# GloryyrolG/MHEntropy

Hardware: AMD Instinct MI355X
Metric: hypotheses/sec (BxK) fwd+loss, 256x256 (higher is better)
Workload: dtype bf16; 1 GPU; c2: MHEnt.get_loss forward+loss, resnet50 encoder (train-mode BN), 12-coupling RealNVP h=512, MANO joints, B=256/GPU, K=64, 256x256; images_per_gpu=256, hypotheses_per_image=64, global_batch=256, launch=hip-graph replay, base_noise=drawn on the device inside the step (Philox4x32-10, mhe_randn_f32), timing=one window of 452 steps, bracketed by barrier + synchronize, ranks=1, rccl_ranks=0

## Files before the change

### mhentropy_amd/csrc/conv_halo.hip

```cpp
#include "conv_shared.h"

#ifndef MHE_HALO_ABL
#define MHE_HALO_ABL 0
#endif

namespace mhe { namespace conv {

namespace {

typedef unsigned u4 __attribute__((ext_vector_type(4)));
typedef __attribute__((ext_vector_type(8))) __bf16 bf8;
typedef float v16f __attribute__((ext_vector_type(16)));

constexpr int HBM = 256, HBN = 128;
constexpr int H_STAGE = 16384, H_RING = 4;
constexpr int H_MAXC = 512;
constexpr unsigned H_OOB = 0x80000000u;

template <int W> struct Geo {
    static constexpr int R = HBM / W;
    static constexpr int PW = W + 2, HP = (R + 2) * PW;
    static constexpr int HALO = HP * 128;
    static constexpr int NP = HP * 8;
    static constexpr int NJ = (NP + 255) / 256;
};

}

template <int W, bool DG>
__global__ __launch_bounds__(768) void conv_halo_kernel(const Params p) {
    using T = u16;
    using G = Geo<W>;
    constexpr int R = G::R, PW = G::PW, HALO = G::HALO, NP = G::NP, NJ = G::NJ;
    static_assert(NJ <= 12, "six load steps of two pieces");
    __shared__ uint4 lds[(H_RING * H_STAGE + 2 * HALO) / 16];
    __shared__ float aff[3 * H_MAXC];
    unsigned char *const ring = reinterpret_cast<unsigned char *>(lds), *const halo0 = ring + H_RING * H_STAGE;
    const int tid = threadIdx.x, lane = tid & 63, wave = __builtin_amdgcn_readfirstlane(tid >> 6);
    const int C = p.Cin, nC = C / 64, Tn = nC * 9;
    const int gm = p.M / HBM, gn = p.Cout / HBN, ntiles = gm * gn;
    const int TPI = p.H / R;
    auto tile_at = [&](int L, int &mt, int &nt) __attribute__((always_inline)) {
        if (gn > 1 && (gm & 7) == 0) {
            const int slot = L >> 3;
            nt = slot % gn;
            mt = (slot / gn) * 8 + (L & 7);
        } else { mt = L % gm; nt = L / gm; }
    };
    const bool bn = p.in_scale != nullptr;
    const bool rev = DG && p.rev_coef != nullptr;
    if (rev) for (int i = tid; i < C; i += 768) { aff[i] = p.rev_coef[i]; aff[H_MAXC + i] = p.rev_coef[C + i]; aff[2 * H_MAXC + i] = p.rev_coef[2 * C + i]; }
    constexpr int abl = MHE_HALO_ABL;
    if (bn) for (int i = tid; i < C; i += 768) { aff[i] = p.in_scale[i]; aff[H_MAXC + i] = p.in_shift[i]; }
    const int nbar_epi = (MHE_HALO_ABL & 16) ? 3 : 3 + (!DG && p.stats ? 2 : 0) + (DG && BN_EPILOGUE && p.bn_y[0] ? 2 : 0);
    __syncthreads();

    if (wave < 8) {
        const int l31 = lane & 31, kg = lane >> 5;
        const int wm = wave >> 1, wn = wave & 1;
        int hpb[2], xcb[2];
#pragma unroll
        for (int mt = 0; mt < 2; ++mt) {
            const int pm = wm * 64 + mt * 32 + l31;
            hpb[mt] = (pm / W + 1) * PW + (pm % W) + 1;
            xcb[mt] = (pm % W) + 1;
        }
        const size_t wbytes = (size_t)gn * Tn * H_STAGE;
        const u4 rsw = {(unsigned)(size_t)p.w, (unsigned)((size_t)p.w >> 32) & 0xffffu, (unsigned)wbytes, 0x00020000u};
        const unsigned ring_lds = (unsigned)(size_t)((__attribute__((address_space(3))) unsigned char *)ring);
        int gc = 0;
        for (int L = blockIdx.x; L < ntiles; L += (int)gridDim.x) {
            int mtile, ntile;
            tile_at(L, mtile, ntile);
            auto issue = [&](int tau) __attribute__((always_inline)) {
                const unsigned off = tau < Tn ? (unsigned)((ntile * Tn + tau) * H_STAGE + wave * 2048 + lane * 16) : H_OOB;
                const unsigned off1 = tau < Tn ? off + 1024u : H_OOB;
                const unsigned lb = ring_lds + (unsigned)((tau & 3) * H_STAGE + wave * 2048);
                unsigned keep;
                asm volatile("s_mov_b32 %[keep], m0\n\ts_mov_b32 m0, %[lb]\n\ts_nop 0\n\tbuffer_load_dwordx4 %[v0], %[rs], 0 offen lds\n\t"
                             "s_add_u32 m0, %[lb], 1024\n\ts_nop 0\n\tbuffer_load_dwordx4 %[v1], %[rs], 0 offen lds\n\ts_mov_b32 m0, %[keep]"
                             : [keep] "=&s"(keep) : [v0] "v"(off), [v1] "v"(off1), [rs] "s"(rsw), [lb] "s"(lb) : "memory");
            };
            v16f acc[2][2];
#pragma unroll
            for (int a = 0; a < 2; ++a)
#pragma unroll
                for (int b = 0; b < 2; ++b)
#pragma unroll
                    for (int i = 0; i < 16; ++i) acc[a][b][i] = 0.f;
            if constexpr (!(abl & 4)) { issue(0); issue(1); issue(2); }
            __builtin_amdgcn_s_barrier();
            __builtin_amdgcn_sched_barrier(0);
            for (int c = 0; c < nC; ++c) {
                const unsigned char *hb = halo0 + ((gc + c) & 1) * HALO;
#pragma unroll
                for (int tap = 0; tap < 9; ++tap) {
                    const int tau = c * 9 + tap;
                    asm volatile("s_waitcnt vmcnt(4)" ::: "memory");
                    __builtin_amdgcn_s_barrier();
                    __builtin_amdgcn_sched_barrier(0);
                    if constexpr (!(abl & 4)) issue(tau + 3);
                    if constexpr (abl & 2) continue;
                    const unsigned char *ws = ring + ((c + tap) & 3) * H_STAGE + (wn * 8) * 1024 + lane * 16;
                    const int toff = (tap / 3 - 1) * PW + (tap % 3 - 1);
                    const unsigned char *ha[2];
                    int fx[2];
#pragma unroll
                    for (int mt = 0; mt < 2; ++mt) {
                        int hp0 = hpb[mt];
                        asm volatile("" : "+v"(hp0));
                        const int hp = hp0 + toff;
                        ha[mt] = hb + hp * 128;
                        fx[mt] = (kg ^ (((xcb[mt] + (tap % 3 - 1)) >> 1) & 7)) << 4;
                    }
#pragma unroll
                    for (int ks = 0; ks < 4; ++ks) {
                        uint4 fb[2], fa[2];
#pragma unroll
                        for (int nt = 0; nt < 2; ++nt) fb[nt] = *reinterpret_cast<const uint4 *>(ws + (nt * 4 + ks) * 1024);
#pragma unroll
                        for (int mt = 0; mt < 2; ++mt) fa[mt] = *reinterpret_cast<const uint4 *>(ha[mt] + (fx[mt] ^ (ks << 5)));
#pragma unroll
                        for (int nt = 0; nt < 2; ++nt)
#pragma unroll
                            for (int mt = 0; mt < 2; ++mt)
                                if constexpr (abl & 1) acc[nt][mt][0] += __uint_as_float((fb[nt].x ^ fa[mt].x) + (fb[nt].w ^ fa[mt].w));
                                else acc[nt][mt] = __builtin_amdgcn_mfma_f32_32x32x16_bf16(__builtin_bit_cast(bf8, fb[nt]), __builtin_bit_cast(bf8, fa[mt]),
                                                                                           acc[nt][mt], 0, 0, 0);
                    }
                }
            }
            gc += nC;
            asm volatile("s_waitcnt vmcnt(0)" ::: "memory");
            __builtin_amdgcn_s_barrier();
            __builtin_amdgcn_sched_barrier(0);
#pragma unroll
            for (int nt = 0; nt < 2; ++nt)
#pragma unroll
                for (int mt = 0; mt < 2; ++mt)
#pragma unroll
                    for (int b = 0; b < 4; ++b) {
                        const int row = wm * 64 + mt * 32 + l31, boff = (wn * 64 + nt * 32 + 8 * b + 4 * kg) * 2;
                        const int chunk = (boff >> 4) ^ (row & 15);
                        uint2 o;
                        o.x = (unsigned)f32_to_bf16(acc[nt][mt][4 * b]) | ((unsigned)f32_to_bf16(acc[nt][mt][4 * b + 1]) << 16);
                        o.y = (unsigned)f32_to_bf16(acc[nt][mt][4 * b + 2]) | ((unsigned)f32_to_bf16(acc[nt][mt][4 * b + 3]) << 16);
                        *reinterpret_cast<uint2 *>(ring + ((size_t)row * 16 + chunk) * 16 + (boff & 15)) = o;
                    }
            __syncthreads();
            const int m0 = mtile * HBM;
            if constexpr (!(abl & 16)) epilogue_store<T, HBM, HBN, 512, DG, 2, 1>(p, ring, mtile % NSH, ntile * HBN, [&](int row) { return (long)(m0 + row); });
            __syncthreads();
        }
    } else {
        const int tr = tid - 512;
        const T *xg = reinterpret_cast<const T *>(p.x);
        auto locate = [&](int j, int rb, int r1, int cc, long &goff, int &lo, bool &inner) __attribute__((always_inline)) {
            int trv = tr;
            asm volatile("" : "+v"(trv));
            const int e = trv + 256 * j;
            if (e >= NP) { goff = -2; lo = 0; inner = false; return; }
            const int hp = e >> 3, slot = e & 7, hr = hp / PW, hc = hp - hr * PW;
            const int col = hc - 1;
            lo = hp * 128 + ((slot ^ ((hc >> 1) & 7)) << 4);
            const bool ok = (unsigned)(r1 + hr) < (unsigned)p.H && (unsigned)col < (unsigned)W;
            goff = ok ? ((long)(rb + hr) * W + col) * C + cc * 64 + slot * 8 : -1l;
            inner = ok && hr >= 1 && hr <= R;
        };
        uint4 regs[NJ], regs2[DG ? NJ : 1];
        const T *x2g = reinterpret_cast<const T *>(p.x2);
        const int slot8 = (tr & 7) * 8;
        float sc[8], sh[8], k0[DG ? 8 : 1];
        auto affine_of = [&](int cc) __attribute__((always_inline)) {
#pragma unroll
            for (int i = 0; i < 8; ++i) { sc[i] = aff[cc * 64 + slot8 + i]; sh[i] = aff[H_MAXC + cc * 64 + slot8 + i]; }
            if constexpr (DG) {
#pragma unroll
                for (int i = 0; i < 8; ++i) k0[i] = aff[2 * H_MAXC + cc * 64 + slot8 + i];
            }
        };
        auto load_all = [&](int rb, int r1, int cc) __attribute__((always_inline)) {
#pragma unroll
            for (int j = 0; j < NJ; ++j) {
                long goff; int lo; bool inner;
                locate(j, rb, r1, cc, goff, lo, inner);
                regs[j] = goff >= 0 ? *reinterpret_cast<const uint4 *>(xg + goff) : make_uint4(0u, 0u, 0u, 0u);
                if constexpr (DG) { if (rev) regs2[j] = goff >= 0 ? *reinterpret_cast<const uint4 *>(x2g + goff) : make_uint4(0u, 0u, 0u, 0u); }
            }
        };
        auto store2 = [&](int s, int rb, int r1, int cc, unsigned char *hb, T *ag) __attribute__((always_inline)) {
#pragma unroll
            for (int i = 0; i < 2; ++i) {
                const int j = 2 * s + i;
                if (j >= NJ) continue;
                long goff; int lo; bool inner;
                locate(j, rb, r1, cc, goff, lo, inner);
                if (goff == -2) continue;
                uint4 v = regs[j];
                if (bn && goff >= 0) {
                    float f[8];
                    Chunk<T>::unpack(v, f);
#pragma unroll
                    for (int k = 0; k < 8; ++k) { f[k] = fmaf(f[k], sc[k], sh[k]); if (p.relu_in) f[k] = fmaxf(f[k], 0.f); }
                    v = Chunk<T>::pack(f);
                }
                if constexpr (DG) {
                    if (rev && goff >= 0) {
                        float f[8], y[8];
                        Chunk<T>::unpack(v, f);
                        Chunk<T>::unpack(regs2[j], y);
#pragma unroll
                        for (int k = 0; k < 8; ++k) f[k] = fmaf(sc[k], f[k], fmaf(sh[k], y[k], k0[k]));
                        v = Chunk<T>::pack(f);
                    }
                }
                *reinterpret_cast<uint4 *>(hb + lo) = v;
                if (ag && inner) *reinterpret_cast<uint4 *>(ag + goff) = v;
            }
        };
        int gc = 0;
        {
            int mt0, nt0;
            tile_at(blockIdx.x, mt0, nt0);
            T *ag = p.a_out && nt0 == 0 ? reinterpret_cast<T *>(p.a_out) : nullptr;
            const int r1 = (mt0 % TPI) * R - 1, rb = (mt0 / TPI) * p.H + r1;
            if (bn || rev) affine_of(0);
            load_all(rb, r1, 0);
#pragma unroll
            for (int s = 0; s < 6; ++s) store2(s, rb, r1, 0, halo0, ag);
        }
        for (int L = blockIdx.x; L < ntiles; L += (int)gridDim.x) {
            int mtile, ntile;
            tile_at(L, mtile, ntile);
            for (int c = 0; c < nC; ++c) {
                int mt2 = mtile, nt2 = ntile, c2 = c + 1;
                bool have = true;
                if (c2 == nC) {
                    c2 = 0;
                    have = L + (int)gridDim.x < ntiles;
                    if (have) tile_at(L + (int)gridDim.x, mt2, nt2);
                }
                unsigned char *hb = halo0 + ((gc + c + 1) & 1) * HALO;
                T *ag = p.a_out && nt2 == 0 ? reinterpret_cast<T *>(p.a_out) : nullptr;
                const int r1 = (mt2 % TPI) * R - 1, rb = (mt2 / TPI) * p.H + r1;
                if (c == 0) {
                    asm volatile("s_waitcnt lgkmcnt(0)" ::: "memory");
                    __builtin_amdgcn_s_barrier();
                    __builtin_amdgcn_sched_barrier(0);
                }
#pragma unroll
                for (int s = 0; s < 9; ++s) {
                    if (have && !(abl & 8)) {
                        if (s == 0) { load_all(rb, r1, c2); if (bn || rev) affine_of(c2); }
                        if (s >= 3) store2(s - 3, rb, r1, c2, hb, ag);
                    }
                    asm volatile("s_waitcnt lgkmcnt(0)" ::: "memory");
                    __builtin_amdgcn_s_barrier();
                    __builtin_amdgcn_sched_barrier(0);
                }
            }
            gc += nC;
            asm volatile("s_waitcnt lgkmcnt(0)" ::: "memory");
            for (int i = 0; i < nbar_epi; ++i) __builtin_amdgcn_s_barrier();
        }
    }
}

bool halo_supports(const Params &p) {
    return p.KH == 3 && p.KW == 3 && p.stride == 1 && p.pad == 1 && (p.W == 32 || p.W == 16) && p.H % (HBM / p.W) == 0 && p.Cin % 64 == 0 &&
           p.Cin >= 64 && p.Cin <= H_MAXC && p.Cout % HBN == 0 && p.M % HBM == 0 && (!p.x2 || (p.mask && p.rev_coef && !p.in_scale)) && !p.os2 && !p.res_s2 && !p.y32 && !p.xcat &&
           !(p.mask && p.stats) && (size_t)(p.Cout / HBN) * (p.Cin / 64) * 9 * H_STAGE < 0x7fff0000ull;
}

int launch_halo(const Params &p, hipStream_t s) {
    const int ntiles = (p.M / HBM) * (p.Cout / HBN);
    const dim3 grid((unsigned)(ntiles < 256 ? ntiles : 256)), block(768);
    if (p.W == 32) {
        if (p.mask) hipLaunchKernelGGL((conv_halo_kernel<32, true>), grid, block, 0, s, p);
        else hipLaunchKernelGGL((conv_halo_kernel<32, false>), grid, block, 0, s, p);
    } else {
        if (p.mask) hipLaunchKernelGGL((conv_halo_kernel<16, true>), grid, block, 0, s, p);
        else hipLaunchKernelGGL((conv_halo_kernel<16, false>), grid, block, 0, s, p);
    }
    return check_launch("conv_halo_kernel");
}

__global__ void halo_pack_kernel(const u16 *w, u16 *out, int Cout, int Cin, int Kpad) {
    const long n = (long)(Cout / HBN) * (Cin / 64) * 9 * 16 * 64;
    const long i = (long)blockIdx.x * blockDim.x + threadIdx.x;
    if (i >= n) return;
    const int lane = (int)(i & 63), f = (int)((i >> 6) & 15);
    const long st = i >> 10;
    const int tap = (int)(st % 9), c = (int)((st / 9) % (Cin / 64)), ntile = (int)(st / 9 / (Cin / 64));
    const int cout = ntile * HBN + (f >> 2) * 32 + (lane & 31), k = tap * Cin + c * 64 + (f & 3) * 16 + (lane >> 5) * 8;
    *reinterpret_cast<uint4 *>(out + i * 8) = *reinterpret_cast<const uint4 *>(w + (size_t)cout * Kpad + k);
}

}}

using namespace mhe;

static bool halo_geometry(conv::Params &p, int B, int H, int W, int Cin, int Cout) {
    const mhe_conv_desc d = {B, H, W, Cin, Cout, 3, 3, 1, 1, MHE_BF16};
    p.force = -1;
    return conv::fill_geometry(p, d) < (1ll << 31) && B > 0 && H > 0 && W > 0;
}

extern "C" int mhe_conv3x3_halo_supported(int B, int H, int W, int Cin, int Cout) {
    conv::Params p{};
    return halo_geometry(p, B, H, W, Cin, Cout) && conv::halo_supports(p) ? 1 : 0;
}

extern "C" int mhe_conv3x3_halo_pack_bf16(const void *w, void *w_halo, int Cout, int Cin, void *stream) {
    MHE_REQUIRE(w && w_halo, "mhe_conv3x3_halo_pack_bf16: null pointer");
    MHE_REQUIRE(Cout > 0 && Cout % 128 == 0 && Cin > 0 && Cin % 64 == 0, "mhe_conv3x3_halo_pack_bf16: Cout %% 128 and Cin %% 64 must be 0");
    const long n = (long)(Cout / 128) * (Cin / 64) * 9 * 16 * 64;
    hipLaunchKernelGGL(conv::halo_pack_kernel, dim3((unsigned)((n + 255) / 256)), dim3(256), 0, (hipStream_t)stream, (const u16 *)w, (u16 *)w_halo, Cout,
                       Cin, 9 * Cin);
    return check_launch("halo_pack_kernel");
}

extern "C" int mhe_conv3x3_halo_nhwc(int B, int H, int W, int Cin, int Cout, const void *x, const void *w_halo, void *y, const float *in_scale,
                                     const float *in_shift, int relu_in, void *a_out, mhe_stat_t *stats, const void *residual, const void *mask,
                                     const void *bn_y0, const float *bn_mean_invstd0, mhe_stat_t *bn_stats0, void *stream) {
    MHE_REQUIRE(x && w_halo && y, "mhe_conv3x3_halo_nhwc: null pointer");
    MHE_REQUIRE((in_scale == nullptr) == (in_shift == nullptr), "mhe_conv3x3_halo_nhwc: in_scale/in_shift must come together");
    MHE_REQUIRE(!a_out || in_scale, "mhe_conv3x3_halo_nhwc: a_out is the normalised operand: it needs in_scale / in_shift");
    MHE_REQUIRE(!(mask && stats) && !(residual && !mask), "mhe_conv3x3_halo_nhwc: statistics in the forward form, residual in the data-gradient form only");
    MHE_REQUIRE(!bn_y0 || (mask && bn_mean_invstd0 && bn_stats0), "mhe_conv3x3_halo_nhwc: bn_y needs the gate, its mean_invstd and stats");
    conv::Params p{};
    p.x = x; p.w = w_halo; p.y = y; p.in_scale = in_scale; p.in_shift = in_shift; p.relu_in = relu_in; p.a_out = a_out; p.stats = stats;
    p.residual = residual; p.mask = mask; p.bn_y[0] = bn_y0; p.bn_mi[0] = bn_mean_invstd0; p.bn_stats[0] = bn_stats0;
    MHE_REQUIRE(halo_geometry(p, B, H, W, Cin, Cout), "mhe_conv3x3_halo_nhwc: bad geometry");
    MHE_REQUIRE(conv::halo_supports(p), "mhe_conv3x3_halo_nhwc: geometry not taken (3x3 stride 1 pad 1, W 32 / 16, Cin %% 64, Cin <= 512, Cout %% 128)");
    return conv::launch_halo(p, (hipStream_t)stream);
}

extern "C" int mhe_conv3x3_halo_dgrad_bn_nhwc(int B, int H, int W, int Cin, int Cout, const void *g, const void *y_raw, const float *coef, const void *w_halo,
                                              void *gx, void *gy_out, const void *residual, const void *mask, const void *bn_y0,
                                              const float *bn_mean_invstd0, mhe_stat_t *bn_stats0, void *stream) {
    MHE_REQUIRE(g && y_raw && coef && w_halo && gx && mask, "mhe_conv3x3_halo_dgrad_bn_nhwc: null pointer");
    MHE_REQUIRE(!bn_y0 || (bn_mean_invstd0 && bn_stats0), "mhe_conv3x3_halo_dgrad_bn_nhwc: bn_y needs its mean_invstd and stats");
    conv::Params p{};
    p.x = g; p.x2 = y_raw; p.rev_coef = coef; p.w = w_halo; p.y = gx; p.a_out = gy_out;
    p.residual = residual; p.mask = mask; p.bn_y[0] = bn_y0; p.bn_mi[0] = bn_mean_invstd0; p.bn_stats[0] = bn_stats0;
    MHE_REQUIRE(halo_geometry(p, B, H, W, Cin, Cout), "mhe_conv3x3_halo_dgrad_bn_nhwc: bad geometry");
    MHE_REQUIRE(conv::halo_supports(p), "mhe_conv3x3_halo_dgrad_bn_nhwc: geometry not taken (see mhe_conv3x3_halo_nhwc)");
    return conv::launch_halo(p, (hipStream_t)stream);
}
```

### mhentropy_amd/switches.py

```python
import os

SWITCHES = {
    "MHE_CONV_TILE": ("-1", "csrc/conv.hip", "force convolution variant k where the geometry admits it (tuning runs)"),
    "MHE_CONV_STREAM": ("1", "csrc/conv.hip", "0: no streaming 1x1 / row-streaming 3x3 kernels (variants 8 / 9)"),
    "MHE_CONV_WIDE": ("1", "csrc/conv.hip", "0: no resident-slab kernel (variant 11)"),
    "MHE_CONV_TAIL": ("1", "csrc/conv.hip", "0: no residual-tail kernel with transfer waves (variant 10)"),
    "MHE_CONV_P8H": ("1", "csrc/conv.hip", "0: no 256x128 phase-pipelined tile (variant 13)"),
    "MHE_CONV_HALO": ("1", "resnet.py, train.py", "0: 3x3 stride-1 units of layer2 / layer3 on the im2col kernels instead of the resident-tile kernel"),
    "MHE_BN_APPLY": ("pass", "resnet.py", "pass | load: where a producer's BatchNorm + ReLU is applied by default"),
    "MHE_BN_APPLY_1X1": ("auto", "resnet.py", "pass | load | auto for the 1x1 consumers"),
    "MHE_BN_APPLY_3X3": ("auto", "resnet.py", "pass | load | auto for the 3x3 consumers"),
    "MHE_BN_LOAD_S2": ("256", "resnet.py", "BatchNorm on the load of the stride-2 3x3 launches up to this many channels"),
    "MHE_FUSE_TAIL": ("1", "resnet.py", "0: block tails as separate bn_act passes"),
    "MHE_FUSE_RECOMPUTE": ("1", "resnet.py", "0: conv3 of layer1 / layer2 written and read back (forward-only path)"),
    "MHE_RECOMPUTE_STATS": ("gram", "resnet.py", "stream: bn3 statistics from the statistics-only launch instead of the Gram matrix"),
    "MHE_STEM_POOL": ("1", "resnet.py", "0: stem convolution and max pool as two kernels"),
    "MHE_FUSE_POOL": ("1", "resnet.py", "0: last block tail and average pool as two launches"),
    "MHE_STAGE_ENTRY": ("1", "resnet.py", "0: stage-entry tails write the whole block output, the stride-2 shortcut reads it, bn3 / shortcut finalized by two launches"),
    "MHE_GRAM_WGS_64": ("512", "csrc/conv_gram.hip", "workgroups of the 64-channel Gram launch"),
    "MHE_GRAM_WGS_128": ("256", "csrc/conv_gram.hip", "workgroups of the 128-channel Gram launch"),
    "MHE_FLOW_FRAG": ("1", "flows.py, train_flow.py", "0: second-generation coupling-stack kernel (flow_ns.hip) instead of the fragment-streaming one"),
    "MHE_FLOW_W1_SETS": ("2", "csrc/flow_fwd.hip", "3: a third register set of layer-1 weight fragments (measured equal)"),
    "MHE_GLOW_FUSED": ("1", "glow.py, train_glow.py", "0: the Glow branch's sampling pass layer by layer (~60 launches) instead of the one-launch kernel"),
    "MHE_GLOW_REV_FUSED": ("1", "train_glow.py", "0: the Glow branch's reverse pass over the tape stage by stage instead of the one-launch chain (csrc/glow_rev.hip)"),
    "MHE_MANO_FOUR": ("1", "csrc/mano.hip", "0: one hypothesis per wavefront"),
    "MHE_LBS_MFMA": ("1", "body.py", "0: the body model's skinning with one thread per vertex (csrc/body.hip) instead of the matrix-core kernel (csrc/lbs_skin.hip)"),
    "MHE_MANO_SKIN_MFMA": ("1", "csrc/mano.hip", "0: full-mesh skinning with one thread per vertex (round 1) instead of the matrix-core kernel on bf16 pieces (csrc/mano_skin.hip)"),
    "MHE_TRAIN_RECOMPUTE": ("1", "train.py", "0: conv3 of layer1 / layer2 written by the train step's forward pass"),
    "MHE_CONV3_FOLD": ("1", "train.py", "0: conv3 + bn3 reversed by reading y3 (no Gram fold)"),
    "MHE_CONV3_FOLD_CAT": ("1", "train.py", "0: the fold's second product as a launch of its own"),
    "MHE_SHORTCUT_FOLD": ("1", "train.py", "0: layer1's shortcut reversed by the apply pass"),
    "MHE_STEM_BWD_TWO_PASS": ("1", "train.py", "0: the stem's scattered pool gradient written and read back"),
    "MHE_STEM_POOL_FUSED": ("1", "train.py", "0: stem BatchNorm + ReLU not folded into its max pool"),
    "MHE_STEM_POOLED_SUMS": ("1", "train.py", "0: the stem's BatchNorm-reverse sums from a walk over its full-resolution output"),
    "MHE_STEM_WGRAD_PAIRS": ("1", "train.py", "0: the stem's weight gradient over single pixels (3 channels padded to 8)"),
    "MHE_GATE_BITS": ("1", "train.py", "0: ReLU gates read from the block-wide tensors instead of their bits"),
    "MHE_CONV_HALO_DG": ("1", "train.py", "0: 3x3 data gradients on the im2col kernels"),
    "MHE_HALO_BN_ON_LOAD": ("0", "train.py", "1: the unit's BatchNorm reverse on the resident-tile data-gradient launch's load (measured equal)"),
    "MHE_BN_REDUCE_FUSED": ("1", "train.py", "0: BatchNorm-reverse sums in a pass of their own"),
    "MHE_BN_BWD_ON_LOAD": ("1", "train.py", "0: BatchNorm-reverse apply always as a pass"),
    "MHE_BN_BWD_ON_LOAD_MAXC": ("128", "train.py", "widest bottleneck whose conv3 reverse takes the apply on its operand load"),
    "MHE_BN_BWD_ON_LOAD_WIDE": ("1", "train.py", "0: layer3 / layer4's conv3 reverse without the apply on its load"),
    "MHE_BN_BWD_APPLY_WIDE": ("1", "csrc/trunk_bwd.hip", "0: 8-byte lanes in the apply pass"),
    "MHE_COND_BWD_BF16": ("1", "train.py", "0: the conditioning projections' reverse products on f32 operands"),
    "MHE_FLOW_WGRAD_GROUPED": ("1", "train_flow.py", "0: one weight-gradient launch per coupling net"),
    "MHE_FLOW_REV_FUSED": ("1", "train_flow.py", "0: the flow's reverse chain coupling by coupling"),
    "MHE_FLOW_RECOMPUTE": ("0", "train_flow.py", "1: the reverse pass re-evaluates the flow nets instead of reading emitted activations"),
    "MHE_LAZY_FALLBACK_TABLES": ("1", "arena.py", "0: the fallback operand layouts refreshed every step"),
    "MHE_POISON_STALE_TABLES": ("0", "arena.py", "1 (debug): fallback operand layouts a repack leaves behind are filled with NaN"),
    "MHE_GATHER_AFFINE": ("1", "arena.py", "0: the bf16 operand re-pack from one index per element instead of (base, stride, validity) per eight"),
    "MHE_WGRAD_MULTI": ("1", "train.py", "0: one weight-gradient launch per trunk layer instead of one multi-problem launch per gradient bucket and tile shape"),
    "MHE_WGRAD_MULTI_WGS": ("2048", "csrc/wgrad.hip", "workgroups a multi-problem launch of the 4-wave tiles aims at"),
    "MHE_WGRAD_MULTI_WGS_BIG": ("768", "csrc/wgrad.hip", "workgroups a multi-problem launch of the 256 x 256 tile aims at"),
    "MHE_WGRAD_W16": ("1", "csrc/wgrad.hip", "0: the 256 x 256 weight-gradient tile on eight waves of 64 x 128 instead of sixteen of 64 x 64"),
    "MHE_WGRAD_DMA": ("1", "csrc/wgrad.hip", "0: register-staged bf16 weight-gradient kernel"),
    "MHE_WGRAD_BIG": ("1", "csrc/wgrad.hip", "0: no 256x256 weight-gradient tile"),
    "MHE_WGRAD_XCD": ("1", "csrc/wgrad.hip", "0: weight-gradient tiles in grid order"),
    "MHE_WGRAD_WGS": ("512", "csrc/wgrad.hip", "target workgroup count of a split launch"),
    "MHE_WGRAD_MINCHUNK": ("512", "csrc/wgrad.hip", "shortest pixel slice of the bf16 kernels"),
    "MHE_WGRAD_SLABS": ("all", "csrc/wgrad.hip", "big: small layers add their tiles with f32 atomics (order-dependent sums)"),
    "MHE_WGRAD_F32MFMA": ("", "csrc/wgrad.hip", "set: bf16 operands through the f32 MFMA kernel"),
    "MHE_GRAD_EXCHANGE": ("f32", "dist.py", "bf16: gradient buckets exchanged as bf16 (all-to-all + all-gather, f32 accumulation) instead of an f32 all-reduce"),
    "MHE_DIST_FORCE": ("0", "dist.py", "1: issue every collective in a group of ONE rank (one-GPU rehearsal of the RCCL path)"),
    "MHE_BENCH_REHEARSE": ("0", "bench.py", "1: all ranks share cuda:0 and talk over gloo (development only)"),
}


def non_default(environ=None):
    env = os.environ if environ is None else environ
    return {k: env[k] for k, (default, _, _) in SWITCHES.items() if k in env and env[k] != default}


def markdown_table():
    rows = ["| variable | default | read by | non-default value selects |", "|---|---|---|---|"]
    rows += [f"| `{k}` | `{d or '(unset)'}` | `{w}` | {m} |" for k, (d, w, m) in SWITCHES.items()]
    return "\n".join(rows)


if __name__ == "__main__":
    print(markdown_table())
```

Measured before the change: 2.625 million hypotheses/s.

## Overlap halo conv output write-out with next tile's halo loads

In the forward form of the resident-tile 3x3 conv kernel, half of each tile's output (one wn half) is now staged into the free halo buffer. It is written to global memory, with BatchNorm statistics accumulated, during the first load steps of the next tile instead of in a serial epilogue. The other half is still walked immediately. The aim is to hide epilogue store latency behind the next tile's loads. This adds register pressure, extra barriers and LDS reuse hazards. It is enabled by default only for the 16-wide maps with more than 256 tiles.

```diff
diff --git a/mhentropy_amd/csrc/conv_halo.hip b/mhentropy_amd/csrc/conv_halo.hip
--- a/mhentropy_amd/csrc/conv_halo.hip
+++ b/mhentropy_amd/csrc/conv_halo.hip
@@ -25,12 +25,41 @@
     static constexpr int NJ = (NP + 255) / 256;
 };
 
-}
-
-template <int W, bool DG>
+__device__ __forceinline__ void halo_walk_half(const Params &p, const unsigned char *st, int t, size_t m0, int nh, bool st_on, float *ss1, float *ss2, int j0,
+                                               int j1) {
+    u16 *yg = reinterpret_cast<u16 *>(p.y);
+    asm volatile("" : "+v"(t));
+    const int c = t & 7, r0 = t >> 3;
+#pragma unroll
+    for (int j = j0; j < j1; ++j) {
+        const int row = r0 + 32 * j;
+        const uint4 raw = *reinterpret_cast<const uint4 *>(st + ((size_t)row * 8 + (c ^ (row & 7))) * 16);
+        if (st_on) {
+            float sv[8];
+            Chunk<u16>::unpack(raw, sv);
+#pragma unroll
+            for (int i = 0; i < 8; ++i) { ss1[i] += sv[i]; ss2[i] = fmaf(sv[i], sv[i], ss2[i]); }
+        }
+        *reinterpret_cast<uint4 *>(yg + (m0 + row) * p.Cout + nh + c * 8) = raw;
+    }
+}
+
+__device__ __forceinline__ void halo_fold_half(const Params &p, const float *red, int q, int shard, int nh) {
+    const int c = q >> 3, e = q & 7;
+    float a = 0.f, b = 0.f;
+    for (int k = 0; k < 32; ++k) { a += red[(c + 8 * k) * 16 + e]; b += red[(c + 8 * k) * 16 + 8 + e]; }
+    fx::add(p.stats, shard, 0, p.Cout, nh + q, a);
+    fx::add(p.stats, shard, 1, p.Cout, nh + q, b);
+}
+
+}
+
+template <int W, bool DG, bool OV = false>
 __global__ __launch_bounds__(768) void conv_halo_kernel(const Params p) {
     using T = u16;
     using G = Geo<W>;
+    static_assert(!(OV && DG), "the overlapped walk is the forward form's");
+    constexpr bool OVL = OV && MHE_HALO_ABL == 0;
     constexpr int R = G::R, PW = G::PW, HALO = G::HALO, NP = G::NP, NJ = G::NJ;
     static_assert(NJ <= 12, "six load steps of two pieces");
     __shared__ uint4 lds[(H_RING * H_STAGE + 2 * HALO) / 16];
@@ -134,6 +163,42 @@
             asm volatile("s_waitcnt vmcnt(0)" ::: "memory");
             __builtin_amdgcn_s_barrier();
             __builtin_amdgcn_sched_barrier(0);
+            if constexpr (OVL) {
+                if (L + (int)gridDim.x < ntiles) {
+                    unsigned char *const st = wn ? ring : halo0 + ((gc - 1) & 1) * HALO;
+#pragma unroll
+                    for (int nt = 0; nt < 2; ++nt)
+#pragma unroll
+                        for (int mt = 0; mt < 2; ++mt)
+#pragma unroll
+                            for (int b = 0; b < 4; ++b) {
+                                const int row = wm * 64 + mt * 32 + l31, boff = (nt * 32 + 8 * b + 4 * kg) * 2;
+                                const int chunk = (boff >> 4) ^ (row & 7);
+                                uint2 o;
+                                o.x = (unsigned)f32_to_bf16(acc[nt][mt][4 * b]) | ((unsigned)f32_to_bf16(acc[nt][mt][4 * b + 1]) << 16);
+                                o.y = (unsigned)f32_to_bf16(acc[nt][mt][4 * b + 2]) | ((unsigned)f32_to_bf16(acc[nt][mt][4 * b + 3]) << 16);
+                                *reinterpret_cast<uint2 *>(st + ((size_t)row * 8 + chunk) * 16 + (boff & 15)) = o;
+                            }
+                    __syncthreads();
+                    const bool st_on = p.stats != nullptr;
+                    float ss1[8], ss2[8];
+#pragma unroll
+                    for (int i = 0; i < 8; ++i) ss1[i] = ss2[i] = 0.f;
+                    if (wave < 4) halo_walk_half(p, ring, tid, (size_t)mtile * HBM, ntile * HBN + 64, st_on, ss1, ss2, 0, 8);
+                    if (st_on) {
+                        float *red = reinterpret_cast<float *>(ring);
+                        __syncthreads();
+                        if (wave < 4) {
+#pragma unroll
+                            for (int i = 0; i < 8; ++i) { red[tid * 16 + i] = ss1[i]; red[tid * 16 + 8 + i] = ss2[i]; }
+                        }
+                        __syncthreads();
+                        if (wave == 0) halo_fold_half(p, red, tid, mtile % NSH, ntile * HBN + 64);
+                    }
+                    __syncthreads();
+                    continue;
+                }
+            }
 #pragma unroll
             for (int nt = 0; nt < 2; ++nt)
 #pragma unroll
@@ -218,6 +283,12 @@
                 if (ag && inner) *reinterpret_cast<uint4 *>(ag + goff) = v;
             }
         };
+        float ws1[OVL ? 8 : 1], ws2[OVL ? 8 : 1];
+        const unsigned char *wst = nullptr;
+        size_t wm0 = 0;
+        int wnh = 0, wshard = 0;
+        bool wk = false;
+        const bool st_on = p.stats != nullptr;
         int gc = 0;
         {
             int mt0, nt0;
@@ -254,6 +325,7 @@
                         if (s == 0) { load_all(rb, r1, c2); if (bn || rev) affine_of(c2); }
                         if (s >= 3) store2(s - 3, rb, r1, c2, hb, ag);
                     }
+                    if constexpr (OVL) { if (wk && c == 0 && s < 3) halo_walk_half(p, wst, tr, wm0, wnh, st_on, ws1, ws2, 3 * s, s == 2 ? 8 : 3 * s + 3); }
                     asm volatile("s_waitcnt lgkmcnt(0)" ::: "memory");
                     __builtin_amdgcn_s_barrier();
                     __builtin_amdgcn_sched_barrier(0);
@@ -261,7 +333,31 @@
             }
             gc += nC;
             asm volatile("s_waitcnt lgkmcnt(0)" ::: "memory");
-            for (int i = 0; i < nbar_epi; ++i) __builtin_amdgcn_s_barrier();
+            if constexpr (OVL) {
+                const bool pend = wk && st_on;
+                const bool ovt = L + (int)gridDim.x < ntiles;
+                unsigned char *const pfree = halo0 + ((gc - 1) & 1) * HALO;
+                float *const red = reinterpret_cast<float *>(ovt ? ring + 2 * H_STAGE : pfree);
+                __builtin_amdgcn_s_barrier();
+                __builtin_amdgcn_sched_barrier(0);
+                if (pend) {
+#pragma unroll
+                    for (int i = 0; i < 8; ++i) { red[tr * 16 + i] = ws1[i]; red[tr * 16 + 8 + i] = ws2[i]; }
+                }
+                asm volatile("s_waitcnt lgkmcnt(0)" ::: "memory");
+                __builtin_amdgcn_s_barrier();
+                __builtin_amdgcn_sched_barrier(0);
+                if (pend && tr < 64) halo_fold_half(p, red, tr, wshard, wnh);
+                asm volatile("s_waitcnt lgkmcnt(0)" ::: "memory");
+                for (int i = 2; i < nbar_epi; ++i) __builtin_amdgcn_s_barrier();
+                __builtin_amdgcn_sched_barrier(0);
+                wk = ovt;
+                wst = pfree; wm0 = (size_t)mtile * HBM; wnh = ntile * HBN; wshard = mtile % NSH;
+#pragma unroll
+                for (int i = 0; i < 8; ++i) ws1[i] = ws2[i] = 0.f;
+            } else {
+                for (int i = 0; i < nbar_epi; ++i) __builtin_amdgcn_s_barrier();
+            }
         }
     }
 }
@@ -275,11 +371,15 @@
 int launch_halo(const Params &p, hipStream_t s) {
     const int ntiles = (p.M / HBM) * (p.Cout / HBN);
     const dim3 grid((unsigned)(ntiles < 256 ? ntiles : 256)), block(768);
+    const int overlap = getenv("MHE_CONV_HALO_OVERLAP") ? atoi(getenv("MHE_CONV_HALO_OVERLAP")) : 1;
+    const bool ov = (overlap == 2 || (overlap == 1 && p.W == 16)) && !p.mask && ntiles > 256;
     if (p.W == 32) {
         if (p.mask) hipLaunchKernelGGL((conv_halo_kernel<32, true>), grid, block, 0, s, p);
+        else if (ov) hipLaunchKernelGGL((conv_halo_kernel<32, false, true>), grid, block, 0, s, p);
         else hipLaunchKernelGGL((conv_halo_kernel<32, false>), grid, block, 0, s, p);
     } else {
         if (p.mask) hipLaunchKernelGGL((conv_halo_kernel<16, true>), grid, block, 0, s, p);
+        else if (ov) hipLaunchKernelGGL((conv_halo_kernel<16, false, true>), grid, block, 0, s, p);
         else hipLaunchKernelGGL((conv_halo_kernel<16, false>), grid, block, 0, s, p);
     }
     return check_launch("conv_halo_kernel");
diff --git a/mhentropy_amd/switches.py b/mhentropy_amd/switches.py
--- a/mhentropy_amd/switches.py
+++ b/mhentropy_amd/switches.py
@@ -7,6 +7,7 @@
     "MHE_CONV_TAIL": ("1", "csrc/conv.hip", "0: no residual-tail kernel with transfer waves (variant 10)"),
     "MHE_CONV_P8H": ("1", "csrc/conv.hip", "0: no 256x128 phase-pipelined tile (variant 13)"),
     "MHE_CONV_HALO": ("1", "resnet.py, train.py", "0: 3x3 stride-1 units of layer2 / layer3 on the im2col kernels instead of the resident-tile kernel"),
+    "MHE_CONV_HALO_OVERLAP": ("1", "csrc/conv_halo.hip", "0: the resident-tile kernel's forward form walks every tile's output before the next tile starts; 2: the overlapped walk on the 32-wide maps too (read per launch)"),
     "MHE_BN_APPLY": ("pass", "resnet.py", "pass | load: where a producer's BatchNorm + ReLU is applied by default"),
     "MHE_BN_APPLY_1X1": ("auto", "resnet.py", "pass | load | auto for the 1x1 consumers"),
     "MHE_BN_APPLY_3X3": ("auto", "resnet.py", "pass | load | auto for the 3x3 consumers"),
```

Result: no change. 2.615 million hypotheses/s (-0.4%).
